# LordLiang/DrawingSpinUp

Hardware: AMD Instinct MI355X
Metric: drawings/sec end-to-end (512x512, 6 views, 24 frames) (higher is better)
Workload: dtype f16 (diffusion) / f16 table + f32 MLP (NSR) / f32 (stage-1 deformable convolutions, IS-Net, contour) / f32 with bf16 x 3 products (stage-2 convolutions; the reference: cuDNN TF32)

## Files before the change

### drawingspinup_amd/csrc/hashgrid_mfma.hip

```cpp
#include "hashgrid_dev.h"
#include "partial_reduce.h"

#include <type_traits>

using namespace dsu_hg;

namespace {

typedef float f32x16 __attribute__((ext_vector_type(16)));
typedef __bf16 bf16x8 __attribute__((ext_vector_type(8)));

__device__ __forceinline__ void softplus_inplace2(f32x16& acc, int r) {
  const f32x2 h = softplus100_pair(f32x2{acc[r], acc[r + 1]});
  acc[r] = h.x;
  acc[r + 1] = h.y;
}

__device__ __forceinline__ void bf16_split8(const float* x, bf16x8& hi, bf16x8& mid) {
#pragma unroll
  for (int i = 0; i < 8; ++i) {
    const __bf16 h = (__bf16)x[i];
    hi[i] = h;
    mid[i] = (__bf16)(x[i] - (float)h);
  }
}

template <int NL>
struct MC {
  static constexpr int DIN = 3 + 2 * NL;
  static constexpr int KIN = 2 * NL + 4;
  static constexpr int KP = KIN / 2;
};

template <int NL>
// ... 454 lines not shown

  __syncthreads();
  float* red = lds + W1P_F;
  {
    float* r0 = red + wave * PART_STRIDE;
#pragma unroll
    for (int T = 0; T < 2; ++T)
#pragma unroll
      for (int r = 0; r < 16; ++r) {
        const int feat = feat_of(T, r, h);
        float c0 = gw1c0[T][r];
#pragma unroll
        for (int off = 16; off > 0; off >>= 1) c0 += __shfl_xor(c0, off);
        r0[PART_GW0 + feat * 32 + l31] = gw0[T][r];
        r0[PART_GW1 + feat * 32 + l31] = gw1[T][r] + (l31 == 0 ? c0 : 0.0f);
      }
#pragma unroll
    for (int o = 0; o < NOUT; ++o) gb1[o] += __shfl_xor(gb1[o], 32);
#pragma unroll
    for (int off = 16; off > 0; off >>= 1)
#pragma unroll
      for (int o = 0; o < NOUT; ++o) gb1[o] += __shfl_xor(gb1[o], off);
    if (lane == 0) {
#pragma unroll
      for (int o = 0; o < NOUT; ++o) r0[PART_GB1 + o] = gb1[o];
    }
  }
  __syncthreads();
  float* part = partials + (size_t)blockIdx.x * PART_STRIDE;
  for (int v = threadIdx.x; v < PART_GB1 + NOUT; v += blockDim.x)
    part[v] = (red[v] + red[PART_STRIDE + v]) + (red[2 * PART_STRIDE + v] + red[3 * PART_STRIDE + v]);
}

constexpr int PT_ROW = 40;
constexpr int PT_IMGD = 2 * 64 * PT_ROW, PT_IMGI = 2 * 32 * PT_ROW;
constexpr int PIPE_IMG_F = (PT_IMGD + PT_IMGI) / 2;
constexpr int PW_W0 = 0;
constexpr int PW_W1T = PW_W0 + 2 * 9 * 64;
constexpr int PW_W0T = PW_W1T + 2 * 2 * 64 * 4;
constexpr int PW_W1O0 = PW_W0T + 2 * 2 * 2 * 64 * 4;
constexpr int PW_F = PW_W1O0 + 64;
constexpr int PIPE_LDS_F = PW_F + 4 * PIPE_IMG_F;
static_assert(PIPE_LDS_F * sizeof(float) <= 80 * 1024, "two workgroups per CU");
static_assert(4 * PART_STRIDE <= PIPE_LDS_F, "the workgroup reduction reuses the LDS");
static_assert(PW_W1T % 4 == 0 && PW_W0T % 4 == 0 && PW_F % 4 == 0, "16-byte fragments");

template <int NL, int ACT>
__global__ __launch_bounds__(256) __attribute__((amdgpu_waves_per_eu(ACT <= 6 ? 2 : 1))) void sdf_fd_bwd_pipe_kernel(
    dsu_sdf_mlp mlp, const float* __restrict__ pts, int64_t n, float radius, float eps, float eps2,
    const float* __restrict__ d_sdf, const float* __restrict__ d_grad,
    const float* __restrict__ d_feature, const float* __restrict__ d_laplace,
    float* __restrict__ partials, const __half2* __restrict__ enc, float2* __restrict__ dinbuf,
    const int32_t* __restrict__ perm) {
  static_assert(ACT >= 1 && ACT <= NL && 2 * NL + 4 <= 32, "layout");
  constexpr int KPA = ACT + 2;
  static_assert(KPA <= 9, "layer-0 weights fit their LDS slot");
  auto gw1_col = [](int o) { return o < 8 ? 2 * NL + 4 + o : 2 * ACT + (o - 8); };
  static_assert(2 * NL + 4 + 8 == 32 && 2 * ACT + NOUT - 8 <= 2 * NL, "gW1 columns free of inputs");
  constexpr bool L0BF = 2 * KPA <= 16;
  __shared__ __attribute__((aligned(16))) float lds[PIPE_LDS_F];
  const int lane = threadIdx.x & 63, wave = threadIdx.x >> 6;
  const int l31 = lane & 31, h = lane >> 5;
  int wo = 0;
  auto weights_per_use = [&]() {};
  const bf16x8* wfrag = reinterpret_cast<const bf16x8*>(lds);
  auto frag_of = [&](int float_off, int idx) { return wfrag[wo + float_off / 4 + idx * 64 + lane]; };

  if (blockIdx.x == 0 && threadIdx.x == 0)
    *reinterpret_cast<int*>(dinbuf + (size_t)7 * (size_t)n * NL) = 0;

  {
    bf16x8* wst = reinterpret_cast<bf16x8*>(lds);
    if (wave == 0) {
      if constexpr (L0BF) {
#pragma unroll
        for (int T = 0; T < 2; ++T) {
          float w[8];
#pragma unroll
          for (int t = 0; t < 8; ++t) {
            const int j = 8 * h + t, tt = j >> 1;
            const bool real = j < 2 * KPA;
            const int t_ = tt < ACT ? tt : NL + (tt - ACT);
            const float v = w0p<NL>(mlp, 32 * T + l31, real ? 2 * t_ + (j & 1) : 0);
            w[t] = real ? v : 0.0f;
          }
          bf16x8 hi, mid;
          bf16_split8(w, hi, mid);
          wst[PW_W0 / 4 + (2 * T + 0) * 64 + lane] = hi;
          wst[PW_W0 / 4 + (2 * T + 1) * 64 + lane] = mid;
        }
      } else {
#pragma unroll
        for (int T = 0; T < 2; ++T)
// ... 4 lines not shown
          }
      }
    } else if (wave == 1) {
#pragma unroll
      for (int T = 0; T < 2; ++T) {
        float w[8];
#pragma unroll
        for (int t = 0; t < 8; ++t) {
          const int o = 8 * h + t;
          const float v = mlp.w1[(o < NOUT ? o : 0) * 64 + 32 * T + l31];
          w[t] = o < NOUT ? v : 0.0f;
        }
        bf16x8 hi, mid;
        bf16_split8(w, hi, mid);
        wst[PW_W1T / 4 + (2 * T + 0) * 64 + lane] = hi;
        wst[PW_W1T / 4 + (2 * T + 1) * 64 + lane] = mid;
      }
      lds[PW_W1O0 + lane] = mlp.w1[lane];
    } else {
      const int T = wave - 2;
      float w0t[16];
#pragma unroll
      for (int r = 0; r < 16; ++r)
        w0t[r] = l31 < MC<NL>::KIN ? w0p<NL>(mlp, feat_of(T, r, h), l31) : 0.0f;
#pragma unroll
      for (int g = 0; g < 2; ++g) {
        bf16x8 hi, mid;
        bf16_split8(&w0t[8 * g], hi, mid);
        wst[PW_W0T / 4 + ((2 * T + g) * 2 + 0) * 64 + lane] = hi;
        wst[PW_W0T / 4 + ((2 * T + g) * 2 + 1) * 64 + lane] = mid;
      }
    }
  }
  __bf16* imgD = reinterpret_cast<__bf16*>(lds + PW_F + wave * PIPE_IMG_F);
  __bf16* imgI = imgD + PT_IMGD;
  for (int t = lane; t < PT_IMGI / 2; t += 64) reinterpret_cast<uint32_t*>(imgI)[t] = 0u;
  __syncthreads();

  f32x16 gw0[2];
#pragma unroll
  for (int T = 0; T < 2; ++T)
#pragma unroll
    for (int r = 0; r < 16; ++r) gw0[T][r] = 0.0f;
  float gb1[NOUT];
#pragma unroll
  for (int o = 0; o < NOUT; ++o) gb1[o] = 0.0f;

  auto l0_half = [&](const float (&in)[2 * KPA], int half, f32x16 (&acc)[2]) {
    float b[KPA];
#pragma unroll
    for (int tt = 0; tt < KPA; ++tt) {
      float b0, b1;
      swap_halves(in[2 * tt], in[2 * tt + 1], b0, b1);
      b[tt] = half ? b1 : b0;
    }
#pragma unroll
    for (int T = 0; T < 2; ++T) {
#pragma unroll
      for (int r = 0; r < 16; ++r) acc[T][r] = 0.0f;
#pragma unroll
      for (int tt = 0; tt < KPA; ++tt)
        acc[T] = __builtin_amdgcn_mfma_f32_32x32x2f32(lds[wo + PW_W0 + (T * KPA + tt) * 64 + lane], b[tt],
                                                      acc[T], 0, 0, 0);
    }
  };
  typedef uint32_t u32x4 __attribute__((ext_vector_type(4)));
  auto pack_operands = [&](const float* in, auto nc, bf16x8& bh0, bf16x8& bm0, bf16x8& bh1, bf16x8& bm1) {
    constexpr int NV = decltype(nc)::value;
    uint32_t ph[8], pm[8];
// ... 17 lines not shown
    bh0 = __builtin_bit_cast(bf16x8, a0); bh1 = __builtin_bit_cast(bf16x8, a1);
    bm0 = __builtin_bit_cast(bf16x8, c0); bm1 = __builtin_bit_cast(bf16x8, c1);
  };
  auto l0_bf = [&](const bf16x8& bh, const bf16x8& bm, f32x16 (&acc)[2]) {
#pragma unroll
    for (int T = 0; T < 2; ++T) {
#pragma unroll
      for (int r = 0; r < 16; ++r) acc[T][r] = 0.0f;
      const bf16x8 ah = frag_of(PW_W0, 2 * T), am = frag_of(PW_W0, 2 * T + 1);
      acc[T] = __builtin_amdgcn_mfma_f32_32x32x16_bf16(ah, bh, acc[T], 0, 0, 0);
      acc[T] = __builtin_amdgcn_mfma_f32_32x32x16_bf16(ah, bm, acc[T], 0, 0, 0);
      acc[T] = __builtin_amdgcn_mfma_f32_32x32x16_bf16(am, bh, acc[T], 0, 0, 0);
    }
  };
  auto softplus2 = [&](f32x16 (&acc)[2]) {
#pragma unroll
    for (int T = 0; T < 2; ++T)
#pragma unroll
      for (int r = 0; r < 16; r += 2) softplus_inplace2(acc[T], r);
  };
  auto store_din = [&](int e, const f32x16& din, int64_t pi, int64_t r1) {
    if (pi < r1) {
#pragma unroll
      for (int r = 0; r < 16; r += 2) {
        const int la = ((r & 3) + 8 * (r >> 2)) / 2;
        const int lev = la + 2 * h;
        if (la < ACT) {
          if (lev < ACT) dinbuf[((size_t)e * ACT + lev) * n + pi] = make_float2(din[r], din[r + 1]);
        }
      }
    }
  };
  auto stage_dpre_T = [&](int T, int g, const bf16x8& bh, const bf16x8& bm) {
    __bf16* base = imgD + 4 * h * PT_ROW + l31;
#pragma unroll
    for (int t = 0; t < 8; ++t) {
      const int u = 32 * T + (t & 3) + 8 * (2 * g + (t >> 2));
      base[u * PT_ROW] = bh[t];
      base[(64 + u) * PT_ROW] = bm[t];
    }
  };
  auto din_tile = [&](int T, float (&dpre)[16], const f32x16& H, f32x16& din) {
#pragma unroll
    for (int r = 0; r < 16; ++r)
      dpre[r] *= 1.0f - __builtin_amdgcn_exp2f(H[r] * -144.26950408889634f);
#pragma unroll
    for (int g = 0; g < 2; ++g) {
      bf16x8 bh, bm;
      bf16_split8(&dpre[8 * g], bh, bm);
      const bf16x8 ah = frag_of(PW_W0T, (2 * T + g) * 2), am = frag_of(PW_W0T, (2 * T + g) * 2 + 1);
      din = __builtin_amdgcn_mfma_f32_32x32x16_bf16(ah, bh, din, 0, 0, 0);
      din = __builtin_amdgcn_mfma_f32_32x32x16_bf16(ah, bm, din, 0, 0, 0);
      din = __builtin_amdgcn_mfma_f32_32x32x16_bf16(am, bh, din, 0, 0, 0);
      stage_dpre_T(T, g, bh, bm);
    }
  };
  auto stage_in_T = [&](const float (&in)[2 * KPA]) {
    __bf16* base = imgI + l31;
#pragma unroll
    for (int j = 0; j < 2 * KPA; ++j) {
      const int row = j < 2 * ACT ? j : 2 * NL + (j - 2 * ACT);
      const __bf16 hi = (__bf16)in[j];
      base[row * PT_ROW] = hi;
      base[(32 + row) * PT_ROW] = (__bf16)(in[j] - (float)hi);
    }
  };
  auto gemm_T = [&](f32x16 (&acc)[2], const __bf16* imgB) {
    auto frag = [&](const __bf16* img, int row, int ks) {
      return *reinterpret_cast<const bf16x8*>(img + row * PT_ROW + 16 * ks + 8 * h);
    };
#pragma unroll
    for (int S = 0; S < 4; ++S) {
      const int ks = S >> 1, Ti = S & 1;
      const bf16x8 bh = frag(imgB, l31, ks), bm = frag(imgB + 32 * PT_ROW, l31, ks);
      const bf16x8 ah = frag(imgD, 32 * Ti + l31, ks), am = frag(imgD + 64 * PT_ROW, 32 * Ti + l31, ks);
      acc[Ti] = __builtin_amdgcn_mfma_f32_32x32x16_bf16(ah, bh, acc[Ti], 0, 0, 0);
      acc[Ti] = __builtin_amdgcn_mfma_f32_32x32x16_bf16(ah, bm, acc[Ti], 0, 0, 0);
      acc[Ti] = __builtin_amdgcn_mfma_f32_32x32x16_bf16(am, bh, acc[Ti], 0, 0, 0);
    }
  };

  const int64_t per = ((n + gridDim.x - 1) / gridDim.x + 31) / 32 * 32;
  const int64_t r0 = blockIdx.x * per;
  const int64_t r1 = r0 + per < n ? r0 + per : n;
  for (int64_t bbase = r0; bbase < r1; bbase += blockDim.x) {
    int blk = wave, e_start = 0, e_step = 1;
    {
      const int64_t left = r1 - bbase;
      if (left <= 64) { blk = 0; e_start = wave; e_step = 4; }
      else if (left <= 128) { blk = wave & 1; e_start = wave >> 1; e_step = 2; }
    }
    const int64_t wave_first = bbase + blk * 64;
    if (wave_first >= r1) continue;
    const int64_t i = wave_first + lane;
    const bool valid = i < r1;
    const int64_t ii = valid ? i : r1 - 1;
    const bool live1 = wave_first + 32 < r1;
    const float p[3] = {pts[ii * 3], pts[ii * 3 + 1], pts[ii * 3 + 2]};
    const int64_t gi = perm ? (int64_t)perm[ii] : ii;
    float ds = 0.f, dl = 0.f, dg[3] = {0.f, 0.f, 0.f};
    if (valid) {
      if (d_sdf) ds = d_sdf[gi];
      if (d_laplace) dl = d_laplace[gi];
      if (d_grad) { dg[0] = d_grad[gi * 3]; dg[1] = d_grad[gi * 3 + 1]; dg[2] = d_grad[gi * 3 + 2]; }
    }
    __half2 rw[ACT], rwn[ACT];
    {
      const __half2* row = enc + ((size_t)e_start * n + ii) * ACT;
#pragma unroll
      for (int l = 0; l < ACT; ++l) rw[l] = row[l];
#pragma unroll
// ... 47 lines not shown
      bf16x8 cbh0, cbm0, cbh1, cbm1;
      if constexpr (L0BF)
        pack_operands(in, std::integral_constant<int, (2 * KPA <= 16 ? 2 * KPA : 16)>{}, cbh0, cbm0, cbh1, cbm1);
      bf16x8 dbh0, dbm0, dbh1, dbm1;
      pack_operands(dout, std::integral_constant<int, NOUT>{}, dbh0, dbm0, dbh1, dbm1);
#pragma unroll
      for (int half = 0; half < 2; ++half) {
        if (half == 1 && !live1) break;
        weights_per_use();
        f32x16 Hh[2];
        if constexpr (L0BF) l0_bf(half ? cbh1 : cbh0, half ? cbm1 : cbm0, Hh);
        else l0_half(in, half, Hh);
        softplus2(Hh);
        f32x16 din;
#pragma unroll
        for (int r = 0; r < 16; ++r) din[r] = 0.0f;
#pragma unroll
        for (int T = 0; T < 2; ++T) {
          f32x16 dacc;
#pragma unroll
          for (int r = 0; r < 16; ++r) dacc[r] = 0.0f;
          const bf16x8 bh = half ? dbh1 : dbh0, bm = half ? dbm1 : dbm0;
          const bf16x8 ah = frag_of(PW_W1T, 2 * T), am = frag_of(PW_W1T, 2 * T + 1);
          dacc = __builtin_amdgcn_mfma_f32_32x32x16_bf16(ah, bh, dacc, 0, 0, 0);
          dacc = __builtin_amdgcn_mfma_f32_32x32x16_bf16(ah, bm, dacc, 0, 0, 0);
          dacc = __builtin_amdgcn_mfma_f32_32x32x16_bf16(am, bh, dacc, 0, 0, 0);
          float dpre[16];
#pragma unroll
          for (int r = 0; r < 16; ++r) dpre[r] = dacc[r];
          din_tile(T, dpre, Hh[T], din);
        }
        if (h == half) stage_in_T(in);
        __builtin_amdgcn_wave_barrier();
        gemm_T(gw0, imgI);
        __builtin_amdgcn_wave_barrier();
#pragma unroll
        for (int T = 0; T < 2; ++T)
#pragma unroll
          for (int g = 0; g < 2; ++g) {
            float hv[8];
#pragma unroll
            for (int t = 0; t < 8; ++t) hv[t] = Hh[T][8 * g + t];
            bf16x8 bh, bm;
            bf16_split8(hv, bh, bm);
            stage_dpre_T(T, g, bh, bm);
          }
        if (h == half) {
          __bf16* base = imgI + l31;
#pragma unroll
          for (int j = 0; j < 2 * KPA; ++j) {
            const int row = j < 2 * ACT ? j : 2 * NL + (j - 2 * ACT);
            base[row * PT_ROW] = (__bf16)0.0f;
            base[(32 + row) * PT_ROW] = (__bf16)0.0f;
          }
          const float dl_ = valid ? dl : 0.0f;
#pragma unroll
          for (int o = 0; o < NOUT; ++o) {
            float v = valid && d_feature ? d_feature[gi * NOUT + o] : 0.0f;
            if (o == 0 && valid) v += ds - 6.0f * dl_ / eps2;
            const __bf16 hi = (__bf16)v;
            base[gw1_col(o) * PT_ROW] = hi;
            base[(32 + gw1_col(o)) * PT_ROW] = (__bf16)(v - (float)hi);
          }
        }
        __builtin_amdgcn_wave_barrier();
        gemm_T(gw0, imgI);
        __builtin_amdgcn_wave_barrier();
        if (h == half) {
          __bf16* base = imgI + l31;
#pragma unroll
          for (int o = 0; o < NOUT; ++o) {
            base[gw1_col(o) * PT_ROW] = (__bf16)0.0f;
            base[(32 + gw1_col(o)) * PT_ROW] = (__bf16)0.0f;
          }
        }
        store_din(0, din, wave_first + half * 32 + l31, r1);
      }
      if (e + e_step < 7) handover();
      e += e_step;
    }
    float gw1c0[2][16];
#pragma unroll
    for (int T = 0; T < 2; ++T)
#pragma unroll
      for (int r = 0; r < 16; ++r) gw1c0[T][r] = 0.0f;
    float in[2 * KPA];
    float dout0 = 0.0f;
    float q3[3] = {0.f, 0.f, 0.f};
    auto prep_unpack = [&]() {
#pragma unroll
      for (int l = 0; l < ACT; ++l) {
        const float2 f = __half22float2(rw[l]);
        in[2 * l] = f.x;
        in[2 * l + 1] = f.y;
      }
    };
    auto prep_point = [&](int en) {
      fd_point(p, en, eps, radius, q3);
      in[2 * ACT + 0] = contract(q3[0], radius) * 2.0f + -1.0f;
      in[2 * ACT + 1] = contract(q3[1], radius) * 2.0f + -1.0f;
      in[2 * ACT + 2] = contract(q3[2], radius) * 2.0f + -1.0f;
      in[2 * ACT + 3] = 1.0f;
    };
    auto prep_request = [&](int en) {
      const int e2 = en + e_step < 7 ? en + e_step : 6;
      const __half2* row = enc + ((size_t)e2 * n + ii) * ACT;
// ... 24 lines not shown
      if constexpr (L0BF)
        pack_operands(in, std::integral_constant<int, (2 * KPA <= 16 ? 2 * KPA : 16)>{}, obh0, obm0, obh1, obm1);
#pragma unroll
      for (int half = 0; half < 2; ++half) {
        if (half == 1 && !live1) break;
        weights_per_use();
        const float d0 = half ? d0h1 : d0h0;
        f32x16 Hh[2];
        if constexpr (L0BF) l0_bf(half ? obh1 : obh0, half ? obm1 : obm0, Hh);
        else l0_half(in, half, Hh);
        softplus2(Hh);
#pragma unroll
        for (int T = 0; T < 2; ++T)
#pragma unroll
          for (int r = 0; r < 16; ++r) gw1c0[T][r] = fmaf(Hh[T][r], d0, gw1c0[T][r]);
        f32x16 din;
#pragma unroll
        for (int r = 0; r < 16; ++r) din[r] = 0.0f;
#pragma unroll
        for (int T = 0; T < 2; ++T) {
          float dpre[16];
#pragma unroll
          for (int q = 0; q < 4; ++q) {
            const float4 w = *reinterpret_cast<const float4*>(&lds[wo + PW_W1O0 + 32 * T + 8 * q + 4 * h]);
            dpre[4 * q + 0] = w.x * d0;
            dpre[4 * q + 1] = w.y * d0;
            dpre[4 * q + 2] = w.z * d0;
            dpre[4 * q + 3] = w.w * d0;
          }
          din_tile(T, dpre, Hh[T], din);
        }
        if (h == half) stage_in_T(in);
        __builtin_amdgcn_wave_barrier();
        gemm_T(gw0, imgI);
        __builtin_amdgcn_wave_barrier();
        store_din(e, din, wave_first + half * 32 + l31, r1);
      }
      const int en = e + e_step < 7 ? e + e_step : 6;
      handover();
      prep_unpack();
      prep_point(en);
      prep_request(en);
      prep_dout(en);
    }
#pragma unroll
    for (int T = 0; T < 2; ++T)
#pragma unroll
      for (int r = 0; r < 16; ++r) {
        float c0 = gw1c0[T][r];
#pragma unroll
        for (int off = 16; off > 0; off >>= 1) c0 += __shfl_xor(c0, off);
        if (l31 == gw1_col(0)) gw0[T][r] += c0;
      }
  }

  __syncthreads();
  float* red = lds;
  {
    float* rr = red + wave * PART_STRIDE;
#pragma unroll
    for (int T = 0; T < 2; ++T)
#pragma unroll
      for (int r = 0; r < 16; ++r) {
        const int feat = feat_of(T, r, h);
        const bool input = l31 < 2 * ACT || (l31 >= 2 * NL && l31 < 2 * NL + 4);
        rr[PART_GW0 + feat * 32 + l31] = input ? gw0[T][r] : 0.0f;
        const int o = l31 >= 2 * NL + 4 ? l31 - (2 * NL + 4) : (l31 >= 2 * ACT && l31 < 2 * ACT + NOUT - 8 ? l31 - 2 * ACT + 8 : -1);
// ... 537 lines not shown
```

### drawingspinup_amd/csrc/texture_mlp.hip

```cpp
#include "common.h"

namespace {

typedef float f32x16 __attribute__((ext_vector_type(16)));
typedef __bf16 bf16x8 __attribute__((ext_vector_type(8)));

__device__ __forceinline__ void bf16_split8(const float* x, bf16x8& hi, bf16x8& mid) {
#pragma unroll
  for (int i = 0; i < 8; ++i) {
    const __bf16 hh = (__bf16)x[i];
    hi[i] = hh;
    mid[i] = (__bf16)(x[i] - (float)hh);
  }
}

constexpr int TIN = 16, THID = 64, TOUT = 3;
constexpr int W1_ROW = 65;
constexpr int W0_ROW = 17;
constexpr int L_W1 = 0;
constexpr int L_W0 = L_W1 + THID * W1_ROW;
constexpr int L_W2P = L_W0 + THID * W0_ROW;
constexpr int L_B0 = L_W2P + 2 * TOUT * 32;
constexpr int L_B1 = L_B0 + THID;
constexpr int L_B2 = L_B1 + THID;
constexpr int L_WEND = L_B2 + 8;
constexpr int TROW = 40;
constexpr int TIMG_B = 2 * 64 * TROW;
constexpr int TSML_B = 2 * 20 * TROW;
constexpr int S_X = 0, S_Y = TIMG_B / 2, S_S = TIMG_B;
constexpr int STAGE_F = TIMG_B + TSML_B / 2;
constexpr int IMG1_F = 2 * 8 * 64 * 4, IMG0_F = 2 * 4 * 64 * 4;
constexpr int L_IMG1 = L_WEND + 4 * STAGE_F;
constexpr int L_IMG0 = L_IMG1 + IMG1_F;
constexpr int L_IMGF = L_IMG0 + IMG0_F;
constexpr int BWD_LDS_F = L_IMGF + IMG1_F;
constexpr int P_GW1 = 0, P_GW0 = 64 * 64, P_GW2 = P_GW0 + 64 * 32, P_GB1 = P_GW2 + 64 * 32,
              P_GB2 = P_GB1 + 64, PART_N = P_GB2 + 3, PART_STRIDE = 8320;
constexpr int TEX_MAX_BLOCKS = 256;

__device__ __forceinline__ int feat_of(int T, int r, int h) {
  return 32 * T + (r & 3) + 8 * (r >> 2) + 4 * h;
}

__device__ __forceinline__ void swap_halves(float a, float b, float& o0, float& o1) {
  auto r = __builtin_amdgcn_permlane32_swap(__float_as_uint(a), __float_as_uint(b), false, false);
  o0 = __uint_as_float(r[0]);
  o1 = __uint_as_float(r[1]);
}

__device__ __forceinline__ void load_weights(float* lds, const dsu_tex_mlp& m) {
  for (int i = threadIdx.x; i < THID * THID; i += blockDim.x)
    lds[L_W1 + (i >> 6) * W1_ROW + (i & 63)] = m.w1[i];
  for (int i = threadIdx.x; i < THID * TIN; i += blockDim.x)
    lds[L_W0 + (i >> 4) * W0_ROW + (i & 15)] = m.w0[i];
  for (int i = threadIdx.x; i < 2 * TOUT * 32; i += blockDim.x) {
    const int h = i / (TOUT * 32), o = (i / 32) % TOUT, tr = i & 31;
    lds[L_W2P + i] = m.w2[o * THID + feat_of(tr >> 4, tr & 15, h)];
  }
  for (int i = threadIdx.x; i < THID; i += blockDim.x) {
    lds[L_B0 + i] = m.b0[i];
    lds[L_B1 + i] = m.b1[i];
  }
  for (int i = threadIdx.x; i < TOUT; i += blockDim.x) lds[L_B2 + i] = m.b2[i];
}

// ... 156 lines not shown
        in[4 * q] = v.x; in[4 * q + 1] = v.y; in[4 * q + 2] = v.z; in[4 * q + 3] = v.w;
      }
    }
    float out[TOUT] = {0.0f, 0.0f, 0.0f};
#pragma unroll 1
    for (int a = 0; a < 2; ++a) {
      if (wave_first + a * 32 >= r1) continue;
      f32x16 H0[2], H1[2];
      forward_half(lds, in, a, l31, h, H0, H1);
      if (h1_mask) {
        uint32_t mk = 0u;
#pragma unroll
        for (int T = 0; T < 2; ++T)
#pragma unroll
          for (int r = 0; r < 16; ++r) mk |= (H1[T][r] > 0.0f ? 1u : 0u) << (16 * T + r);
        const int64_t si = wave_first + a * 32 + l31;
        if (si < r1) h1_mask[si * 2 + h] = mk;
      }
      float p[TOUT];
      layer2_partial(lds, H1, h, p);
#pragma unroll
      for (int o = 0; o < TOUT; ++o) {
        const float tot = p[o] + __shfl_xor(p[o], 32);
        if (h == a) out[o] = tot;
      }
    }
    if (valid) {
#pragma unroll
      for (int o = 0; o < TOUT; ++o) rgb[i * TOUT + o] = sigmoidf(out[o] + lds[L_B2 + o]);
    }
  }
}

__device__ __forceinline__ void stage_units_T(__bf16* img, const f32x16 (&X)[2], int l31, int h) {
  __bf16* base = img + 4 * h * TROW + l31;
#pragma unroll
  for (int T = 0; T < 2; ++T)
#pragma unroll
    for (int r = 0; r < 16; ++r) {
      const int u = 32 * T + (r & 3) + 8 * (r >> 2);
      const float x = X[T][r];
      const __bf16 hi = (__bf16)x;
      base[u * TROW] = hi;
      base[(64 + u) * TROW] = (__bf16)(x - (float)hi);
    }
}
__device__ __forceinline__ bf16x8 frag_T(const __bf16* img, int row, int ks, int h) {
  return *reinterpret_cast<const bf16x8*>(img + row * TROW + 16 * ks + 8 * h);
}
template <int NJ>
__device__ __forceinline__ void gemm_samples_T(f32x16 (&acc0)[NJ], f32x16 (&acc1)[NJ], const __bf16* A,
                                               int a_mid, const __bf16* B, int b_mid, int rows_b,
                                               int l31, int h) {
  bf16x8 z;
#pragma unroll
  for (int e = 0; e < 8; ++e) z[e] = (__bf16)0.0f;
#pragma unroll
  for (int ks = 0; ks < 2; ++ks) {
    bf16x8 ah[2], am[2], bh[NJ], bm[NJ];
#pragma unroll
    for (int Ti = 0; Ti < 2; ++Ti) {
      ah[Ti] = frag_T(A, 32 * Ti + l31, ks, h);
      am[Ti] = frag_T(A + a_mid, 32 * Ti + l31, ks, h);
    }
#pragma unroll
    for (int Tj = 0; Tj < NJ; ++Tj) {
      const int row = 32 * Tj + l31;
      const bool real = row < rows_b;
      const bf16x8 vh = frag_T(B, real ? row : 0, ks, h), vm = frag_T(B + b_mid, real ? row : 0, ks, h);
      bh[Tj] = real ? vh : z;
      bm[Tj] = real ? vm : z;
    }
#pragma unroll
    for (int Tj = 0; Tj < NJ; ++Tj) {
      acc0[Tj] = __builtin_amdgcn_mfma_f32_32x32x16_bf16(ah[0], bh[Tj], acc0[Tj], 0, 0, 0);
      acc1[Tj] = __builtin_amdgcn_mfma_f32_32x32x16_bf16(ah[1], bh[Tj], acc1[Tj], 0, 0, 0);
      acc0[Tj] = __builtin_amdgcn_mfma_f32_32x32x16_bf16(ah[0], bm[Tj], acc0[Tj], 0, 0, 0);
      acc1[Tj] = __builtin_amdgcn_mfma_f32_32x32x16_bf16(ah[1], bm[Tj], acc1[Tj], 0, 0, 0);
      acc0[Tj] = __builtin_amdgcn_mfma_f32_32x32x16_bf16(am[0], bh[Tj], acc0[Tj], 0, 0, 0);
      acc1[Tj] = __builtin_amdgcn_mfma_f32_32x32x16_bf16(am[1], bh[Tj], acc1[Tj], 0, 0, 0);
    }
  }
}

struct ShadeOut {
  const float* d_normal;
  float* d_grad;
  float* d_feature;
  int64_t tail;
};

template <bool SHADE, bool L1_MASK = false>
__global__ __launch_bounds__(256) void texture_bwd_kernel(
    dsu_tex_mlp m, const float* __restrict__ x, ShadeIn sh, ShadeOut so,
    const float* __restrict__ rgb, const float* __restrict__ d_rgb, int64_t n,
    float* __restrict__ d_x, float* __restrict__ partials,
    const uint32_t* __restrict__ h1_mask = nullptr) {
  extern __shared__ __attribute__((aligned(16))) float lds[];
  const int lane = threadIdx.x & 63, wave = threadIdx.x >> 6, l31 = lane & 31, h = lane >> 5;
  float* st = lds + L_WEND + wave * STAGE_F;
  __bf16* tX = reinterpret_cast<__bf16*>(st + S_X);
  __bf16* tY = reinterpret_cast<__bf16*>(st + S_Y);
  __bf16* tS = reinterpret_cast<__bf16*>(st + S_S);
  load_weights(lds, m);
  __syncthreads();
  {
    bf16x8* img1 = reinterpret_cast<bf16x8*>(lds + L_IMG1);
    bf16x8* img0 = reinterpret_cast<bf16x8*>(lds + L_IMG0);
    for (int f = threadIdx.x; f < 8 * 64; f += blockDim.x) {
      const int ln = f & 63, c = f >> 6, g = c & 1, Tin = (c >> 1) & 1, To = c >> 2;
      float w[8];
#pragma unroll
      for (int t = 0; t < 8; ++t)
        w[t] = lds[L_W1 + feat_of(Tin, 8 * g + t, ln >> 5) * W1_ROW + 32 * To + (ln & 31)];
      bf16_split8(w, img1[f], img1[8 * 64 + f]);
    }
    for (int f = threadIdx.x; f < 4 * 64; f += blockDim.x) {
      const int ln = f & 63, c = f >> 6, g = c & 1, T = c >> 1;
      float w[8];
#pragma unroll
      for (int t = 0; t < 8; ++t)
        w[t] = (ln & 31) < TIN ? lds[L_W0 + feat_of(T, 8 * g + t, ln >> 5) * W0_ROW + (ln & 31)] : 0.0f;
      bf16_split8(w, img0[f], img0[4 * 64 + f]);
    }
    if constexpr (L1_MASK) {
      bf16x8* imgf = reinterpret_cast<bf16x8*>(lds + L_IMGF);
      for (int f = threadIdx.x; f < 8 * 64; f += blockDim.x) {
        const int ln = f & 63, c = f >> 6, g = c & 1, Tin = (c >> 1) & 1, To = c >> 2;
        float w[8];
#pragma unroll
        for (int t = 0; t < 8; ++t)
          w[t] = lds[L_W1 + (32 * To + (ln & 31)) * W1_ROW + feat_of(Tin, 8 * g + t, ln >> 5)];
        bf16_split8(w, imgf[f], imgf[8 * 64 + f]);
      }
    }
  }
// ... 51 lines not shown
        mk2[a_] = h1_mask[si * 2 + h];
      }
    }
#pragma unroll 1
    for (int a = 0; a < 2; ++a) {
      if (wave_first + a * 32 >= r1) continue;
      f32x16 H0[2], H1[2];
      forward_half<L1_MASK>(lds, in, a, l31, h, H0, H1);
      const uint32_t mk = a ? mk2[1] : mk2[0];
      if constexpr (L1_MASK) {
#pragma unroll
        for (int T = 0; T < 2; ++T)
#pragma unroll
          for (int r = 0; r < 16; ++r) H1[T][r] = ((mk >> (16 * T + r)) & 1u) ? H1[T][r] : 0.0f;
      }
      float dza[TOUT];
#pragma unroll
      for (int o = 0; o < TOUT; ++o) {
        const float other = __shfl_xor(dz[o], 32);
        dza[o] = h == a ? dz[o] : other;
      }
      f32x16 D1[2];
#pragma unroll
      for (int T = 0; T < 2; ++T)
#pragma unroll
        for (int r = 0; r < 16; ++r) {
          float v = 0.0f;
#pragma unroll
          for (int o = 0; o < TOUT; ++o)
            v = fmaf(lds[L_W2P + (h * TOUT + o) * 32 + T * 16 + r], dza[o], v);
          D1[T][r] = (L1_MASK ? ((mk >> (16 * T + r)) & 1u) != 0u : H1[T][r] > 0.0f) ? v : 0.0f;
        }
      __builtin_amdgcn_wave_barrier();
      stage_units_T(tX, H1, l31, h);
      if (h == a) {
#pragma unroll
        for (int o = 0; o < TOUT; ++o) {
          const __bf16 hi = (__bf16)dz[o];
          tS[o * TROW + l31] = hi;
          tS[(20 + o) * TROW + l31] = (__bf16)(dz[o] - (float)hi);
        }
      }
      __builtin_amdgcn_wave_barrier();
      {
        f32x16 (&g0)[1] = *reinterpret_cast<f32x16 (*)[1]>(&gw2[0]);
        f32x16 (&g1)[1] = *reinterpret_cast<f32x16 (*)[1]>(&gw2[1]);
        gemm_samples_T<1>(g0, g1, tX, 64 * TROW, tS, 20 * TROW, TOUT, l31, h);
      }
      __builtin_amdgcn_wave_barrier();
      stage_units_T(tY, D1, l31, h);
      stage_units_T(tX, H0, l31, h);
      __builtin_amdgcn_wave_barrier();
      {
        float srow = 0.0f;
#pragma unroll
        for (int q = 0; q < 4; ++q) {
          const bf16x8 vh = *reinterpret_cast<const bf16x8*>(tY + lane * TROW + 8 * q);
          const bf16x8 vm = *reinterpret_cast<const bf16x8*>(tY + (64 + lane) * TROW + 8 * q);
#pragma unroll
          for (int e = 0; e < 8; ++e) srow += (float)vh[e] + (float)vm[e];
        }
        gb1row += srow;
      }
      gemm_samples_T<2>(gw1[0], gw1[1], tY, 64 * TROW, tX, 64 * TROW, 64, l31, h);
      f32x16 D0[2];
#pragma unroll
      for (int T = 0; T < 2; ++T)
#pragma unroll
        for (int r = 0; r < 16; ++r) D0[T][r] = 0.0f;
      {
        const bf16x8* img1 = reinterpret_cast<const bf16x8*>(lds + L_IMG1);
        bf16x8 bh[2][2], bm[2][2];
#pragma unroll
        for (int Tin = 0; Tin < 2; ++Tin)
#pragma unroll
          for (int g = 0; g < 2; ++g) {
            float v[8];
#pragma unroll
            for (int t = 0; t < 8; ++t) v[t] = D1[Tin][8 * g + t];
            bf16_split8(v, bh[Tin][g], bm[Tin][g]);
          }
#pragma unroll
        for (int To = 0; To < 2; ++To)
#pragma unroll
          for (int Tin = 0; Tin < 2; ++Tin)
#pragma unroll
            for (int g = 0; g < 2; ++g) {
              const int f = ((To * 2 + Tin) * 2 + g) * 64 + lane;
              const bf16x8 ah = img1[f], am = img1[8 * 64 + f];
              D0[To] = __builtin_amdgcn_mfma_f32_32x32x16_bf16(ah, bh[Tin][g], D0[To], 0, 0, 0);
              D0[To] = __builtin_amdgcn_mfma_f32_32x32x16_bf16(ah, bm[Tin][g], D0[To], 0, 0, 0);
              D0[To] = __builtin_amdgcn_mfma_f32_32x32x16_bf16(am, bh[Tin][g], D0[To], 0, 0, 0);
            }
      }
#pragma unroll
      for (int T = 0; T < 2; ++T)
#pragma unroll
        for (int r = 0; r < 16; ++r) D0[T][r] = H0[T][r] > 0.0f ? D0[T][r] : 0.0f;
      __builtin_amdgcn_wave_barrier();
      stage_units_T(tY, D0, l31, h);
      if (h == a) {
#pragma unroll
        for (int k = 0; k < TIN; ++k) {
          const __bf16 hi = (__bf16)in[k];
          tS[k * TROW + l31] = hi;
          tS[(20 + k) * TROW + l31] = (__bf16)(in[k] - (float)hi);
        }
        tS[TIN * TROW + l31] = (__bf16)1.0f;
        tS[(20 + TIN) * TROW + l31] = (__bf16)0.0f;
      }
      __builtin_amdgcn_wave_barrier();
      {
        f32x16 (&g0)[1] = *reinterpret_cast<f32x16 (*)[1]>(&gw0[0]);
        f32x16 (&g1)[1] = *reinterpret_cast<f32x16 (*)[1]>(&gw0[1]);
        gemm_samples_T<1>(g0, g1, tY, 64 * TROW, tS, 20 * TROW, TIN + 1, l31, h);
      }
      f32x16 din;
#pragma unroll
      for (int r = 0; r < 16; ++r) din[r] = 0.0f;
      {
        const bf16x8* img0 = reinterpret_cast<const bf16x8*>(lds + L_IMG0);
#pragma unroll
        for (int T = 0; T < 2; ++T)
#pragma unroll
          for (int g = 0; g < 2; ++g) {
            float v[8];
#pragma unroll
            for (int t = 0; t < 8; ++t) v[t] = D0[T][8 * g + t];
            bf16x8 bh, bm;
            bf16_split8(v, bh, bm);
            const int f = (T * 2 + g) * 64 + lane;
            const bf16x8 ah = img0[f], am = img0[4 * 64 + f];
            din = __builtin_amdgcn_mfma_f32_32x32x16_bf16(ah, bh, din, 0, 0, 0);
            din = __builtin_amdgcn_mfma_f32_32x32x16_bf16(ah, bm, din, 0, 0, 0);
            din = __builtin_amdgcn_mfma_f32_32x32x16_bf16(am, bh, din, 0, 0, 0);
          }
      }
      const int64_t si = wave_first + a * 32 + l31;
      if (si < r1) {
        if (SHADE) {
#pragma unroll
          for (int q = 0; q < 2; ++q)
#pragma unroll
            for (int e = 0; e < 4; ++e) {
              const int comp = 8 * q + 4 * h + e;
              if (comp < 13) so.d_feature[si * 13 + comp] = din[4 * q + e];
            }
          if (h == 1) {
// ... 236 lines not shown
```

Measured before the change: 0.3528.

## Stage MFMA operands with swizzled LDS and ds_read_tr transposed reads

Replaces the padded-row LDS staging images, which used per-element bf16 scalar stores and row-major fragment reads, with a swizzled layout written in 8-byte slots. MFMA operands are then fetched with the ds_read_tr16_b64 transposed-read instruction. Compile-time checks assert the lane address mapping and zero bank conflicts for both stores and reads. The goal is fewer LDS store instructions and fewer bank conflicts in the SDF backward and texture MLP backward kernels. The cost is a more intricate addressing scheme and a dependence on gfx950 transpose-load support.

```diff
diff --git a/drawingspinup_amd/csrc/hashgrid_mfma.hip b/drawingspinup_amd/csrc/hashgrid_mfma.hip
--- a/drawingspinup_amd/csrc/hashgrid_mfma.hip
+++ b/drawingspinup_amd/csrc/hashgrid_mfma.hip
@@ -1,5 +1,6 @@
 #include "hashgrid_dev.h"
 #include "partial_reduce.h"
+#include "tr_stage.h"
 
 #include <type_traits>
 
@@ -520,18 +521,21 @@
     part[v] = (red[v] + red[PART_STRIDE + v]) + (red[2 * PART_STRIDE + v] + red[3 * PART_STRIDE + v]);
 }
 
-constexpr int PT_ROW = 40;
-constexpr int PT_IMGD = 2 * 64 * PT_ROW, PT_IMGI = 2 * 32 * PT_ROW;
-constexpr int PIPE_IMG_F = (PT_IMGD + PT_IMGI) / 2;
+typedef trs::Img<64> ImgD;
+typedef trs::Img<32> ImgI;
+constexpr int PT_IMGD_B = 2 * ImgD::PART_B, PT_IMGI_B = 2 * ImgI::PART_B;
+constexpr int PIPE_IMG_F = (PT_IMGD_B + PT_IMGI_B) / 4;
 constexpr int PW_W0 = 0;
 constexpr int PW_W1T = PW_W0 + 2 * 9 * 64;
 constexpr int PW_W0T = PW_W1T + 2 * 2 * 64 * 4;
 constexpr int PW_W1O0 = PW_W0T + 2 * 2 * 2 * 64 * 4;
 constexpr int PW_F = PW_W1O0 + 64;
-constexpr int PIPE_LDS_F = PW_F + 4 * PIPE_IMG_F;
+constexpr int PIPE_LDS_F = PW_F + 4 * PIPE_IMG_F > 4 * PART_STRIDE ? PW_F + 4 * PIPE_IMG_F : 4 * PART_STRIDE;
 static_assert(PIPE_LDS_F * sizeof(float) <= 80 * 1024, "two workgroups per CU");
 static_assert(4 * PART_STRIDE <= PIPE_LDS_F, "the workgroup reduction reuses the LDS");
 static_assert(PW_W1T % 4 == 0 && PW_W0T % 4 == 0 && PW_F % 4 == 0, "16-byte fragments");
+static_assert(PW_F * 4 % ImgD::ROW_B == 0 && PIPE_IMG_F * 4 % ImgD::ROW_B == 0 && PT_IMGD_B % ImgI::ROW_B == 0,
+              "image bases: multiples of the row (tr_stage.h)");
 
 template <int NL, int ACT>
 __global__ __launch_bounds__(256) __attribute__((amdgpu_waves_per_eu(ACT <= 6 ? 2 : 1))) void sdf_fd_bwd_pipe_kernel(
@@ -546,7 +550,7 @@
   auto gw1_col = [](int o) { return o < 8 ? 2 * NL + 4 + o : 2 * ACT + (o - 8); };
   static_assert(2 * NL + 4 + 8 == 32 && 2 * ACT + NOUT - 8 <= 2 * NL, "gW1 columns free of inputs");
   constexpr bool L0BF = 2 * KPA <= 16;
-  __shared__ __attribute__((aligned(16))) float lds[PIPE_LDS_F];
+  __shared__ __attribute__((aligned(128))) float lds[PIPE_LDS_F];
   const int lane = threadIdx.x & 63, wave = threadIdx.x >> 6;
   const int l31 = lane & 31, h = lane >> 5;
   int wo = 0;
@@ -617,9 +621,18 @@
       }
     }
   }
-  __bf16* imgD = reinterpret_cast<__bf16*>(lds + PW_F + wave * PIPE_IMG_F);
-  __bf16* imgI = imgD + PT_IMGD;
-  for (int t = lane; t < PT_IMGI / 2; t += 64) reinterpret_cast<uint32_t*>(imgI)[t] = 0u;
+  {
+    uint32_t* imgI0 = reinterpret_cast<uint32_t*>(lds + PW_F + wave * PIPE_IMG_F) + PT_IMGD_B / 4;
+    for (int t = lane; t < PT_IMGI_B / 4; t += 64) imgI0[t] = 0u;
+  }
+  const uint32_t ldsD = __builtin_amdgcn_readfirstlane(trs::lds_addr(lds + PW_F + wave * PIPE_IMG_F));
+  const uint32_t ldsI = ldsD + PT_IMGD_B;
+  const uint32_t stD = ldsD + (ImgD::store_base(l31) ^ (8 * h));
+  auto lane_again = [&]() {
+    int l = lane;
+    asm volatile("" : "+v"(l));
+    return l;
+  };
   __syncthreads();
 
   f32x16 gw0[2];
@@ -703,12 +716,11 @@
     }
   };
   auto stage_dpre_T = [&](int T, int g, const bf16x8& bh, const bf16x8& bm) {
-    __bf16* base = imgD + 4 * h * PT_ROW + l31;
-#pragma unroll
-    for (int t = 0; t < 8; ++t) {
-      const int u = 32 * T + (t & 3) + 8 * (2 * g + (t >> 2));
-      base[u * PT_ROW] = bh[t];
-      base[(64 + u) * PT_ROW] = bm[t];
+#pragma unroll
+    for (int q = 0; q < 2; ++q) {
+      const int s = 8 * T + 4 * g + 2 * q;
+      trs::store_slot(stD, s, 0, q ? __builtin_shufflevector(bh, bh, 4, 5, 6, 7) : __builtin_shufflevector(bh, bh, 0, 1, 2, 3));
+      trs::store_slot(stD, s, ImgD::PART_B, q ? __builtin_shufflevector(bm, bm, 4, 5, 6, 7) : __builtin_shufflevector(bm, bm, 0, 1, 2, 3));
     }
   };
   auto din_tile = [&](int T, float (&dpre)[16], const f32x16& H, f32x16& din) {
@@ -726,28 +738,52 @@
       stage_dpre_T(T, g, bh, bm);
     }
   };
+  auto put_cols = [&](uint32_t stI, int s, const float (&v)[4]) {
+    trs::bf16x4 hi, mid;
+#pragma unroll
+    for (int c = 0; c < 4; ++c) {
+      const __bf16 hh = (__bf16)v[c];
+      hi[c] = hh;
+      mid[c] = (__bf16)(v[c] - (float)hh);
+    }
+    trs::store_slot(stI, s, 0, hi);
+    trs::store_slot(stI, s, ImgI::PART_B, mid);
+  };
+  auto in_of_col = [](int col) {
+    return col < 2 * ACT ? col : (col >= 2 * NL && col < 2 * NL + 4 ? 2 * ACT + (col - 2 * NL) : -1);
+  };
+  auto out_of_col = [](int col) {
+    return col >= 2 * NL + 4 ? col - (2 * NL + 4) : (col >= 2 * ACT && col < 2 * ACT + NOUT - 8 ? 8 + (col - 2 * ACT) : -1);
+  };
+  auto store_base_I = [&]() { return ldsI + ImgI::store_base(lane_again() & 31); };
   auto stage_in_T = [&](const float (&in)[2 * KPA]) {
-    __bf16* base = imgI + l31;
-#pragma unroll
-    for (int j = 0; j < 2 * KPA; ++j) {
-      const int row = j < 2 * ACT ? j : 2 * NL + (j - 2 * ACT);
-      const __bf16 hi = (__bf16)in[j];
-      base[row * PT_ROW] = hi;
-      base[(32 + row) * PT_ROW] = (__bf16)(in[j] - (float)hi);
+    const uint32_t stI = store_base_I();
+#pragma unroll
+    for (int s = 0; s < 8; ++s) {
+      float v[4];
+      bool any = false;
+#pragma unroll
+      for (int c = 0; c < 4; ++c) {
+        const int j = in_of_col(4 * s + c);
+        v[c] = j >= 0 ? in[j >= 0 ? j : 0] : 0.0f;
+        any = any || j >= 0;
+      }
+      if (any) put_cols(stI, s, v);
     }
   };
-  auto gemm_T = [&](f32x16 (&acc)[2], const __bf16* imgB) {
-    auto frag = [&](const __bf16* img, int row, int ks) {
-      return *reinterpret_cast<const bf16x8*>(img + row * PT_ROW + 16 * ks + 8 * h);
-    };
-#pragma unroll
-    for (int S = 0; S < 4; ++S) {
-      const int ks = S >> 1, Ti = S & 1;
-      const bf16x8 bh = frag(imgB, l31, ks), bm = frag(imgB + 32 * PT_ROW, l31, ks);
-      const bf16x8 ah = frag(imgD, 32 * Ti + l31, ks), am = frag(imgD + 64 * PT_ROW, 32 * Ti + l31, ks);
-      acc[Ti] = __builtin_amdgcn_mfma_f32_32x32x16_bf16(ah, bh, acc[Ti], 0, 0, 0);
-      acc[Ti] = __builtin_amdgcn_mfma_f32_32x32x16_bf16(ah, bm, acc[Ti], 0, 0, 0);
-      acc[Ti] = __builtin_amdgcn_mfma_f32_32x32x16_bf16(am, bh, acc[Ti], 0, 0, 0);
+  auto gemm_T = [&](f32x16 (&acc)[2]) {
+    const int ln = lane_again();
+    const uint32_t rdD = ldsD + ImgD::read_base(ln), rdI = ldsI + ImgI::read_base(ln);
+#pragma unroll
+    for (int ks = 0; ks < 2; ++ks) {
+      const bf16x8 bh = trs::frag_tr<32>(rdI, ks, 0), bm = trs::frag_tr<32>(rdI, ks, 0, ImgI::PART_B);
+#pragma unroll
+      for (int Ti = 0; Ti < 2; ++Ti) {
+        const bf16x8 ah = trs::frag_tr<64>(rdD, ks, Ti), am = trs::frag_tr<64>(rdD, ks, Ti, ImgD::PART_B);
+        acc[Ti] = __builtin_amdgcn_mfma_f32_32x32x16_bf16(ah, bh, acc[Ti], 0, 0, 0);
+        acc[Ti] = __builtin_amdgcn_mfma_f32_32x32x16_bf16(ah, bm, acc[Ti], 0, 0, 0);
+        acc[Ti] = __builtin_amdgcn_mfma_f32_32x32x16_bf16(am, bh, acc[Ti], 0, 0, 0);
+      }
     }
   };
 
@@ -861,7 +897,7 @@
         }
         if (h == half) stage_in_T(in);
         __builtin_amdgcn_wave_barrier();
-        gemm_T(gw0, imgI);
+        gemm_T(gw0);
         __builtin_amdgcn_wave_barrier();
 #pragma unroll
         for (int T = 0; T < 2; ++T)
@@ -875,32 +911,40 @@
             stage_dpre_T(T, g, bh, bm);
           }
         if (h == half) {
-          __bf16* base = imgI + l31;
-#pragma unroll
-          for (int j = 0; j < 2 * KPA; ++j) {
-            const int row = j < 2 * ACT ? j : 2 * NL + (j - 2 * ACT);
-            base[row * PT_ROW] = (__bf16)0.0f;
-            base[(32 + row) * PT_ROW] = (__bf16)0.0f;
-          }
+          const uint32_t stI = store_base_I();
           const float dl_ = valid ? dl : 0.0f;
+          float dv[NOUT];
 #pragma unroll
           for (int o = 0; o < NOUT; ++o) {
             float v = valid && d_feature ? d_feature[gi * NOUT + o] : 0.0f;
             if (o == 0 && valid) v += ds - 6.0f * dl_ / eps2;
-            const __bf16 hi = (__bf16)v;
-            base[gw1_col(o) * PT_ROW] = hi;
-            base[(32 + gw1_col(o)) * PT_ROW] = (__bf16)(v - (float)hi);
+            dv[o] = v;
+          }
+#pragma unroll
+          for (int s = 0; s < 8; ++s) {
+            float v[4];
+            bool any = false;
+#pragma unroll
+            for (int c = 0; c < 4; ++c) {
+              const int o = out_of_col(4 * s + c);
+              v[c] = o >= 0 ? dv[o >= 0 ? o : 0] : 0.0f;
+              any = any || o >= 0 || in_of_col(4 * s + c) >= 0;
+            }
+            if (any) put_cols(stI, s, v);
           }
         }
         __builtin_amdgcn_wave_barrier();
-        gemm_T(gw0, imgI);
+        gemm_T(gw0);
         __builtin_amdgcn_wave_barrier();
         if (h == half) {
-          __bf16* base = imgI + l31;
-#pragma unroll
-          for (int o = 0; o < NOUT; ++o) {
-            base[gw1_col(o) * PT_ROW] = (__bf16)0.0f;
-            base[(32 + gw1_col(o)) * PT_ROW] = (__bf16)0.0f;
+          const uint32_t stI = store_base_I();
+          const float z[4] = {0.0f, 0.0f, 0.0f, 0.0f};
+#pragma unroll
+          for (int s = 0; s < 8; ++s) {
+            bool any = false;
+#pragma unroll
+            for (int c = 0; c < 4; ++c) any = any || out_of_col(4 * s + c) >= 0;
+            if (any) put_cols(stI, s, z);
           }
         }
         store_din(0, din, wave_first + half * 32 + l31, r1);
@@ -991,7 +1035,7 @@
         }
         if (h == half) stage_in_T(in);
         __builtin_amdgcn_wave_barrier();
-        gemm_T(gw0, imgI);
+        gemm_T(gw0);
         __builtin_amdgcn_wave_barrier();
         store_din(e, din, wave_first + half * 32 + l31, r1);
       }
diff --git a/drawingspinup_amd/csrc/texture_mlp.hip b/drawingspinup_amd/csrc/texture_mlp.hip
--- a/drawingspinup_amd/csrc/texture_mlp.hip
+++ b/drawingspinup_amd/csrc/texture_mlp.hip
@@ -1,4 +1,5 @@
 #include "common.h"
+#include "tr_stage.h"
 
 namespace {
 
@@ -24,13 +25,14 @@
 constexpr int L_B1 = L_B0 + THID;
 constexpr int L_B2 = L_B1 + THID;
 constexpr int L_WEND = L_B2 + 8;
-constexpr int TROW = 40;
-constexpr int TIMG_B = 2 * 64 * TROW;
-constexpr int TSML_B = 2 * 20 * TROW;
-constexpr int S_X = 0, S_Y = TIMG_B / 2, S_S = TIMG_B;
-constexpr int STAGE_F = TIMG_B + TSML_B / 2;
+typedef trs::Img<64> ImgU;
+typedef trs::Img<32> ImgS;
+constexpr int SB_X = 0, SB_Y = 2 * ImgU::PART_B, SB_S = 4 * ImgU::PART_B;
+constexpr int STAGE_F = (4 * ImgU::PART_B + 2 * ImgS::PART_B) / 4;
+constexpr int L_STAGE = (L_WEND + 31) / 32 * 32;
+static_assert(STAGE_F * 4 % ImgU::ROW_B == 0 && SB_S % ImgS::ROW_B == 0, "image bases: multiples of the row");
 constexpr int IMG1_F = 2 * 8 * 64 * 4, IMG0_F = 2 * 4 * 64 * 4;
-constexpr int L_IMG1 = L_WEND + 4 * STAGE_F;
+constexpr int L_IMG1 = L_STAGE + 4 * STAGE_F;
 constexpr int L_IMG0 = L_IMG1 + IMG1_F;
 constexpr int L_IMGF = L_IMG0 + IMG0_F;
 constexpr int BWD_LDS_F = L_IMGF + IMG1_F;
@@ -253,26 +255,39 @@
   }
 }
 
-__device__ __forceinline__ void stage_units_T(__bf16* img, const f32x16 (&X)[2], int l31, int h) {
-  __bf16* base = img + 4 * h * TROW + l31;
+__device__ __forceinline__ void stage_units_T(uint32_t st, const f32x16 (&X)[2]) {
 #pragma unroll
   for (int T = 0; T < 2; ++T)
 #pragma unroll
-    for (int r = 0; r < 16; ++r) {
-      const int u = 32 * T + (r & 3) + 8 * (r >> 2);
-      const float x = X[T][r];
-      const __bf16 hi = (__bf16)x;
-      base[u * TROW] = hi;
-      base[(64 + u) * TROW] = (__bf16)(x - (float)hi);
-    }
-}
-__device__ __forceinline__ bf16x8 frag_T(const __bf16* img, int row, int ks, int h) {
-  return *reinterpret_cast<const bf16x8*>(img + row * TROW + 16 * ks + 8 * h);
+    for (int g = 0; g < 4; ++g) {
+      trs::bf16x4 hi, mid;
+#pragma unroll
+      for (int c = 0; c < 4; ++c) {
+        const float x = X[T][4 * g + c];
+        const __bf16 hh = (__bf16)x;
+        hi[c] = hh;
+        mid[c] = (__bf16)(x - (float)hh);
+      }
+      trs::store_slot(st, 8 * T + 2 * g, 0, hi);
+      trs::store_slot(st, 8 * T + 2 * g, ImgU::PART_B, mid);
+    }
+}
+__device__ __forceinline__ void stage_cols_S(uint32_t st, int s, float v0, float v1, float v2, float v3) {
+  const float v[4] = {v0, v1, v2, v3};
+  trs::bf16x4 hi, mid;
+#pragma unroll
+  for (int c = 0; c < 4; ++c) {
+    const __bf16 hh = (__bf16)v[c];
+    hi[c] = hh;
+    mid[c] = (__bf16)(v[c] - (float)hh);
+  }
+  trs::store_slot(st, s, 0, hi);
+  trs::store_slot(st, s, ImgS::PART_B, mid);
 }
 template <int NJ>
-__device__ __forceinline__ void gemm_samples_T(f32x16 (&acc0)[NJ], f32x16 (&acc1)[NJ], const __bf16* A,
-                                               int a_mid, const __bf16* B, int b_mid, int rows_b,
-                                               int l31, int h) {
+__device__ __forceinline__ void gemm_samples_T(f32x16 (&acc0)[NJ], f32x16 (&acc1)[NJ], uint32_t rdA,
+                                               uint32_t rdB, int cols_b, int l31) {
+  constexpr int CB = 32 * NJ;
   bf16x8 z;
 #pragma unroll
   for (int e = 0; e < 8; ++e) z[e] = (__bf16)0.0f;
@@ -281,14 +296,13 @@
     bf16x8 ah[2], am[2], bh[NJ], bm[NJ];
 #pragma unroll
     for (int Ti = 0; Ti < 2; ++Ti) {
-      ah[Ti] = frag_T(A, 32 * Ti + l31, ks, h);
-      am[Ti] = frag_T(A + a_mid, 32 * Ti + l31, ks, h);
+      ah[Ti] = trs::frag_tr<64>(rdA, ks, Ti);
+      am[Ti] = trs::frag_tr<64>(rdA, ks, Ti, ImgU::PART_B);
     }
 #pragma unroll
     for (int Tj = 0; Tj < NJ; ++Tj) {
-      const int row = 32 * Tj + l31;
-      const bool real = row < rows_b;
-      const bf16x8 vh = frag_T(B, real ? row : 0, ks, h), vm = frag_T(B + b_mid, real ? row : 0, ks, h);
+      const bool real = 32 * Tj + l31 < cols_b;
+      const bf16x8 vh = trs::frag_tr<CB>(rdB, ks, Tj), vm = trs::frag_tr<CB>(rdB, ks, Tj, trs::Img<CB>::PART_B);
       bh[Tj] = real ? vh : z;
       bm[Tj] = real ? vm : z;
     }
@@ -317,12 +331,14 @@
     const float* __restrict__ rgb, const float* __restrict__ d_rgb, int64_t n,
     float* __restrict__ d_x, float* __restrict__ partials,
     const uint32_t* __restrict__ h1_mask = nullptr) {
-  extern __shared__ __attribute__((aligned(16))) float lds[];
+  extern __shared__ __attribute__((aligned(128))) float lds[];
   const int lane = threadIdx.x & 63, wave = threadIdx.x >> 6, l31 = lane & 31, h = lane >> 5;
-  float* st = lds + L_WEND + wave * STAGE_F;
-  __bf16* tX = reinterpret_cast<__bf16*>(st + S_X);
-  __bf16* tY = reinterpret_cast<__bf16*>(st + S_Y);
-  __bf16* tS = reinterpret_cast<__bf16*>(st + S_S);
+  const uint32_t stg = trs::lds_addr(lds + L_STAGE + wave * STAGE_F);
+  const uint32_t stX = stg + SB_X + (ImgU::store_base(l31) ^ (8 * h)), stY = stX + (SB_Y - SB_X);
+  const uint32_t stS = stg + SB_S + ImgS::store_base(l31);
+  const uint32_t rdX = stg + SB_X + ImgU::read_base(lane), rdY = rdX + (SB_Y - SB_X);
+  const uint32_t rdS = stg + SB_S + ImgS::read_base(lane);
+  const uint32_t colY = stg + SB_Y + ImgU::col_base(lane);
   load_weights(lds, m);
   __syncthreads();
   {
@@ -440,37 +456,30 @@
           D1[T][r] = (L1_MASK ? ((mk >> (16 * T + r)) & 1u) != 0u : H1[T][r] > 0.0f) ? v : 0.0f;
         }
       __builtin_amdgcn_wave_barrier();
-      stage_units_T(tX, H1, l31, h);
-      if (h == a) {
-#pragma unroll
-        for (int o = 0; o < TOUT; ++o) {
-          const __bf16 hi = (__bf16)dz[o];
-          tS[o * TROW + l31] = hi;
-          tS[(20 + o) * TROW + l31] = (__bf16)(dz[o] - (float)hi);
-        }
-      }
+      stage_units_T(stX, H1);
+      if (h == a) stage_cols_S(stS, 0, dz[0], dz[1], dz[2], 0.0f);
       __builtin_amdgcn_wave_barrier();
       {
         f32x16 (&g0)[1] = *reinterpret_cast<f32x16 (*)[1]>(&gw2[0]);
         f32x16 (&g1)[1] = *reinterpret_cast<f32x16 (*)[1]>(&gw2[1]);
-        gemm_samples_T<1>(g0, g1, tX, 64 * TROW, tS, 20 * TROW, TOUT, l31, h);
+        gemm_samples_T<1>(g0, g1, rdX, rdS, TOUT, l31);
       }
       __builtin_amdgcn_wave_barrier();
-      stage_units_T(tY, D1, l31, h);
-      stage_units_T(tX, H0, l31, h);
+      stage_units_T(stY, D1);
+      stage_units_T(stX, H0);
       __builtin_amdgcn_wave_barrier();
       {
         float srow = 0.0f;
 #pragma unroll
-        for (int q = 0; q < 4; ++q) {
-          const bf16x8 vh = *reinterpret_cast<const bf16x8*>(tY + lane * TROW + 8 * q);
-          const bf16x8 vm = *reinterpret_cast<const bf16x8*>(tY + (64 + lane) * TROW + 8 * q);
-#pragma unroll
-          for (int e = 0; e < 8; ++e) srow += (float)vh[e] + (float)vm[e];
+        for (int P0 = 0; P0 < 32; P0 += 4) {
+          const uint32_t a4 = (colY ^ (uint32_t)ImgU::col_xor(P0)) + P0 * ImgU::ROW_B;
+          const trs::bf16x4 vh = trs::read_tr(a4), vm = trs::read_tr(a4 + ImgU::PART_B);
+#pragma unroll
+          for (int e = 0; e < 4; ++e) srow += (float)vh[e] + (float)vm[e];
         }
         gb1row += srow;
       }
-      gemm_samples_T<2>(gw1[0], gw1[1], tY, 64 * TROW, tX, 64 * TROW, 64, l31, h);
+      gemm_samples_T<2>(gw1[0], gw1[1], rdY, rdX, 64, l31);
       f32x16 D0[2];
 #pragma unroll
       for (int T = 0; T < 2; ++T)
@@ -506,22 +515,17 @@
 #pragma unroll
         for (int r = 0; r < 16; ++r) D0[T][r] = H0[T][r] > 0.0f ? D0[T][r] : 0.0f;
       __builtin_amdgcn_wave_barrier();
-      stage_units_T(tY, D0, l31, h);
+      stage_units_T(stY, D0);
       if (h == a) {
 #pragma unroll
-        for (int k = 0; k < TIN; ++k) {
-          const __bf16 hi = (__bf16)in[k];
-          tS[k * TROW + l31] = hi;
-          tS[(20 + k) * TROW + l31] = (__bf16)(in[k] - (float)hi);
-        }
-        tS[TIN * TROW + l31] = (__bf16)1.0f;
-        tS[(20 + TIN) * TROW + l31] = (__bf16)0.0f;
+        for (int s = 0; s < TIN / 4; ++s) stage_cols_S(stS, s, in[4 * s], in[4 * s + 1], in[4 * s + 2], in[4 * s + 3]);
+        stage_cols_S(stS, TIN / 4, 1.0f, 0.0f, 0.0f, 0.0f);
       }
       __builtin_amdgcn_wave_barrier();
       {
         f32x16 (&g0)[1] = *reinterpret_cast<f32x16 (*)[1]>(&gw0[0]);
         f32x16 (&g1)[1] = *reinterpret_cast<f32x16 (*)[1]>(&gw0[1]);
-        gemm_samples_T<1>(g0, g1, tY, 64 * TROW, tS, 20 * TROW, TIN + 1, l31, h);
+        gemm_samples_T<1>(g0, g1, rdY, rdS, TIN + 1, l31);
       }
       f32x16 din;
 #pragma unroll
diff --git a/drawingspinup_amd/csrc/tr_stage.h b/drawingspinup_amd/csrc/tr_stage.h
--- /dev/null
+++ b/drawingspinup_amd/csrc/tr_stage.h
@@ -0,0 +1,138 @@
+#pragma once
+#include <stdint.h>
+
+#if defined(__HIPCC__) || defined(__CUDACC__)
+#define TRS_HD __host__ __device__
+#else
+#define TRS_HD
+#endif
+
+namespace trs {
+
+typedef __bf16 bf16x4 __attribute__((ext_vector_type(4)));
+typedef __bf16 bf16x8 __attribute__((ext_vector_type(8)));
+
+template <int COLS>
+struct Img {
+  static_assert(COLS == 32 || COLS == 64, "8 or 16 slots per row");
+  static constexpr int ROW_B = 2 * COLS;
+  static constexpr int SLOTS = COLS / 4;
+  static constexpr int PART_B = 32 * ROW_B;
+
+  TRS_HD static constexpr int swz(int p) {
+    return COLS == 64 ? ((p & 7) | ((((p >> 3) ^ (p >> 1)) & 1) << 3)) : ((p >> 1) & 7);
+  }
+  TRS_HD static constexpr int off(int p, int s) { return p * ROW_B + 8 * (s ^ swz(p)); }
+
+  TRS_HD static constexpr int store_base(int p) { return off(p, 0); }
+
+  TRS_HD static constexpr int read_base(int l) {
+    return off(8 * (l >> 5) + ((l >> 2) & 3), 4 * ((l >> 4) & 1) + (l & 3));
+  }
+  TRS_HD static constexpr int read_xor(int jj, int tile) {
+    return COLS == 64 ? (32 * jj) ^ (64 * tile) : 16 * jj;
+  }
+  TRS_HD static constexpr int read_add(int ks, int jj) { return (16 * ks + 4 * jj) * ROW_B; }
+  TRS_HD static constexpr int read_off(int l, int ks, int jj, int tile) {
+    return (read_base(l) ^ read_xor(jj, tile)) + read_add(ks, jj);
+  }
+
+  TRS_HD static constexpr int col_base(int l) { return off((l >> 2) & 3, 4 * (l >> 4) + (l & 3)); }
+  TRS_HD static constexpr int col_xor(int P0) { return 8 * swz(P0); }
+  TRS_HD static constexpr int col_off(int l, int P0) { return (col_base(l) ^ col_xor(P0)) + P0 * ROW_B; }
+
+  static constexpr bool read_map_ok() {
+    for (int l = 0; l < 64; ++l)
+      for (int ks = 0; ks < 2; ++ks)
+        for (int jj = 0; jj < 2; ++jj)
+          for (int tile = 0; tile < COLS / 32; ++tile) {
+            const int h = l >> 5, c = (l >> 4) & 1, q = (l >> 2) & 3, p = l & 3;
+            if (read_off(l, ks, jj, tile) != off(16 * ks + 8 * h + 4 * jj + q, 8 * tile + 4 * c + p)) return false;
+          }
+    for (int p = 0; p < 32; ++p)
+      for (int s = 0; s < SLOTS; ++s)
+        if ((store_base(p) ^ (8 * s)) != off(p, s)) return false;
+    if (COLS == 64)
+      for (int l = 0; l < 64; ++l)
+        for (int P0 = 0; P0 < 32; P0 += 4)
+          if (col_off(l, P0) != off(P0 + ((l >> 2) & 3), 4 * (l >> 4) + (l & 3))) return false;
+    return true;
+  }
+  static constexpr int extra_cycles(const int (&a)[64], int n, int banks) {
+    int extra = 0;
+    for (int g = 0; g < 64 / n; ++g) {
+      int worst = 1;
+      for (int b = 0; b < banks; ++b) {
+        int cnt = 0, seen[64] = {};
+        for (int i = 0; i < n; ++i)
+          for (int d = 0; d < 2; ++d) {
+            const int dw = a[g * n + i] / 4 + d;
+            if (dw % banks != b) continue;
+            bool dup = false;
+            for (int k = 0; k < cnt; ++k) dup = dup || seen[k] == dw;
+            if (!dup) seen[cnt++] = dw;
+          }
+        worst = cnt > worst ? cnt : worst;
+      }
+      extra += worst - 1;
+    }
+    return extra;
+  }
+  static constexpr int store_conflicts() {
+    int worst = 0;
+    for (int s = 0; s < SLOTS; ++s) {
+      int a[64] = {};
+      for (int l = 0; l < 64; ++l) a[l] = store_base(l & 31) ^ (8 * s);
+      const int e = extra_cycles(a, 16, 32);
+      worst = e > worst ? e : worst;
+    }
+    return worst;
+  }
+  static constexpr int read_conflicts() {
+    int worst = 0;
+    for (int ks = 0; ks < 2; ++ks)
+      for (int jj = 0; jj < 2; ++jj)
+        for (int tile = 0; tile < COLS / 32; ++tile) {
+          int a[64] = {};
+          for (int l = 0; l < 64; ++l) a[l] = read_off(l, ks, jj, tile);
+          const int e = extra_cycles(a, 32, 64);
+          worst = e > worst ? e : worst;
+        }
+    if (COLS == 64)
+      for (int P0 = 0; P0 < 32; P0 += 4) {
+        int a[64] = {};
+        for (int l = 0; l < 64; ++l) a[l] = col_off(l, P0);
+        const int e = extra_cycles(a, 32, 64);
+        worst = e > worst ? e : worst;
+      }
+    return worst;
+  }
+  static_assert(read_map_ok(), "lane addresses of the transposed read");
+  static_assert(store_conflicts() == 0, "ds_write_b64: 0 extra cycles per instruction");
+  static_assert(read_conflicts() == 0, "ds_read_b64_tr_b16: 0 extra cycles per instruction");
+};
+
+#if defined(__HIPCC__)
+#define TRS_LDS __attribute__((address_space(3)))
+__device__ __forceinline__ uint32_t lds_addr(const void* p) {
+  return (uint32_t)(uintptr_t)(TRS_LDS const char*)p;
+}
+__device__ __forceinline__ bf16x4 read_tr(uint32_t a) {
+#if defined(__HIP_DEVICE_COMPILE__)
+  return __builtin_amdgcn_ds_read_tr16_b64_v4bf16((TRS_LDS bf16x4*)(uintptr_t)a);
+#else
+  return bf16x4{};
+#endif
+}
+template <int COLS>
+__device__ __forceinline__ bf16x8 frag_tr(uint32_t rd, int ks, int tile, int add = 0) {
+  const bf16x4 lo = read_tr((rd ^ (uint32_t)Img<COLS>::read_xor(0, tile)) + Img<COLS>::read_add(ks, 0) + add);
+  const bf16x4 hi = read_tr((rd ^ (uint32_t)Img<COLS>::read_xor(1, tile)) + Img<COLS>::read_add(ks, 1) + add);
+  return __builtin_shufflevector(lo, hi, 0, 1, 2, 3, 4, 5, 6, 7);
+}
+__device__ __forceinline__ void store_slot(uint32_t st, int s, int add, bf16x4 v) {
+  *(TRS_LDS bf16x4*)(uintptr_t)((st ^ (uint32_t)(8 * s)) + add) = v;
+}
+#endif
+
+}
```

After: 0.3697, median of 6. 4.8% higher.
